# cr1m5onk1ng/text_similarity

Hardware: AMD Instinct MI355X
Metric: sentences/sec encoded + Mpairs/sec cosine top-k @ N=1M d=384 (higher is better)
Workload: dtype bf16 encoder / f16 selection / fp32 scores

## Files before the change

include/tsim.h:

```cpp
#ifndef TSIM_H
#define TSIM_H

#include <stddef.h>
#include <stdint.h>

#ifdef __cplusplus
extern "C" {
#endif

#define TSIM_OK 0
#define TSIM_EINVAL 1
#define TSIM_EHIP 2
#define TSIM_ENOMEM 3
#define TSIM_EUNSUPPORTED 4

#define TSIM_F32 0
#define TSIM_BF16 1

#define TSIM_ARCH_BERT 0
#define TSIM_ARCH_MPNET 1
#define TSIM_ARCH_ROBERTA 2

int tsim_version(void);
const char *tsim_last_error(void);
// ... 258 lines not shown
void tsim_encoder_destroy(tsim_encoder *enc);

int tsim_encoder_forward(tsim_encoder *enc, const int32_t *tok_ids, const int32_t *tok_pos,
                         const int32_t *tok_col, const int32_t *cu_seqlens, int32_t T, int32_t B,
                         int32_t max_len, float *pooled_f32, void *unit_f16, int ld_unit, float *unit_rho_max,
                         void *last_hidden_bf16, void *stream);

int tsim_encoder_set_token_types(tsim_encoder *enc, const float *type_emb_host, int32_t n_types);
int tsim_encoder_set_cls_head(tsim_encoder *enc, const float *pool_w_host, const float *pool_b_host,
                              const float *cls_w_host, const float *cls_b_host, int32_t num_labels);
int tsim_encoder_set_cls_head_act(tsim_encoder *enc, const float *pool_w_host, const float *pool_b_host,
                                  const float *cls_w_host, const float *cls_b_host, int32_t num_labels, int32_t act);
int tsim_encoder_forward_ex(tsim_encoder *enc, const int32_t *tok_ids, const int32_t *tok_type, const int32_t *tok_pos,
                            const int32_t *tok_col, const int32_t *cu_seqlens, int32_t T, int32_t B, int32_t max_len,
                            float *pooled_f32, void *unit_f16, int ld_unit, float *unit_rho_max,
                            void *last_hidden_bf16, float *logits_f32, void *stream);

#define TSIM_POOL_MEAN 0
#define TSIM_POOL_CLS 1
#define TSIM_POOL_MAX 2
#define TSIM_POOL_MEAN_SQRT_LEN 3
#define TSIM_ACT_IDENTITY 0
#define TSIM_ACT_TANH 1
#define TSIM_ACT_RELU 2
typedef struct tsim_sentence_head {
    int32_t pool_mode;
    int32_t d_out;
    const float *dense_w, *dense_b;
    int32_t dense_act;
    int32_t normalize;
} tsim_sentence_head;

int tsim_encoder_forward_head(tsim_encoder *enc, const int32_t *tok_ids, const int32_t *tok_type, const int32_t *tok_pos,
                              const int32_t *tok_col, const int32_t *cu_seqlens, int32_t T, int32_t B, int32_t max_len,
                              const tsim_sentence_head *head, float *emb_f32, void *unit_f16, int ld_unit,
                              float *unit_rho_max, void *last_hidden_bf16, void *stream);

int tsim_encoder_forward_spans(tsim_encoder *enc, const int32_t *tok_ids, const int32_t *tok_type, const int32_t *tok_pos,
                               const int32_t *tok_col, const int32_t *cu_seqlens, int32_t T, int32_t B, int32_t max_len,
                               float *pooled_f32, void *unit_f16, int ld_unit, float *unit_rho_max,
                               void *last_hidden_bf16, float *logits_f32, const int32_t *span_seq, const int32_t *span_cu,
                               const int32_t *span_tok, int32_t S, int32_t n_span_tok, float *span_out_f32,
                               void *span_unit_f16, int ld_span_unit, float *span_rho_max, void *stream);

#define TSIM_ENC_ERR_TOKEN_ID 1
#define TSIM_ENC_ERR_POSITION 2
#define TSIM_ENC_ERR_MAX_LEN 4
#define TSIM_ENC_ERR_TOKEN_TYPE 8
#define TSIM_ENC_ERR_SPAN 16
int tsim_encoder_error_flags(tsim_encoder *enc, int32_t *flags_host, void *stream);

int tsim_chain_items_host(int blocks, int rem_blocks, int ntiles, int G, int b, int32_t *items, int cap);

#define TSIM_FAMILY_H64 0
#define TSIM_FAMILY_H384_PACKED 1
#define TSIM_FAMILY_H384_ROWMAJOR 2
#define TSIM_FAMILY_PP 3
#define TSIM_FAMILY_PP_MX 4
#define TSIM_ROUTE_QKV 0
#define TSIM_ROUTE_O 1
#define TSIM_ROUTE_FFN1 2
#define TSIM_ROUTE_FFN2 3
#define TSIM_FORM_BF16_128x64 1
#define TSIM_FORM_BF16_128x128 2
#define TSIM_FORM_XRES2 3
#define TSIM_FORM_XRES2_PACKED 4
#define TSIM_FORM_PP_256_PACKED_W 5
#define TSIM_FORM_PP_256 6
#define TSIM_FORM_PP_128 7
#define TSIM_FORM_PP_MX 8
#define TSIM_FORM_BF16_RES_LN 9
#define TSIM_FORM_LN384 10
#define TSIM_FORM_PP_RES_LN_PACKED_W 11
#define TSIM_FORM_PP_RES_LN 12
#define TSIM_FORM_PP_MX_RES_LN 13
#define TSIM_SEG_LN_ROWS 1
#define TSIM_SEG_LN_ROWS_CHAINED 2
#define TSIM_SEG_LN_TAIL 3
#define TSIM_SEG_LN_SPLIT2 4
#define TSIM_SEG_LN_SPLIT4 5
#define TSIM_SEG_BF16_128x384 6
#define TSIM_SEG_BF16_64x384 7
#define TSIM_IMG_PP_QKV_O 1
#define TSIM_IMG_LN_KTILE 2
#define TSIM_IMG_LN_FRAG 4
#define TSIM_IMG_MXFP8 8
#define TSIM_BUF_YBUF 1
#define TSIM_BUF_LNIMG 2
#define TSIM_BUF_MX_ACT 4
#define TSIM_ROUTE_MAX_SEGS 4

typedef struct tsim_route_segment {
    int32_t form, row0, rows;
} tsim_route_segment;

typedef struct tsim_encoder_route {
    int32_t family;
    int32_t form[4];
    int32_t images;
    int32_t buffers;
    int32_t chain_blocks;
    int32_t qkv_chained;
    int32_t n_seg[2];
    tsim_route_segment seg[2][TSIM_ROUTE_MAX_SEGS];
} tsim_encoder_route;

// ... 15 lines not shown
```

text_similarity_amd/_lib.py:

```python
from __future__ import annotations

import ctypes as C
import os

_HERE = os.path.dirname(os.path.abspath(__file__))
LIB_PATH = os.environ.get("TSIM_LIB") or os.path.join(_HERE, "libtsim.so")

TSIM_F32, TSIM_BF16 = 0, 1
TSIM_I32, TSIM_I64 = 2, 3
LIST_ST_ROW, LIST_ST_LIMS = 1, 2
IVF_ST_LIST, IVF_ST_OFF = 1, 2
COMMUNITY_ST_ROW, COMMUNITY_ST_LIMS = 1, 2
IVF_SEG = 512
IVFPQ_SEG = 4096
GRAPH_ST_ROW, GRAPH_ST_ITERS = 1, 2
GRAPH_MAX_TABLE_BYTES = 131072
GRAPH_STATIC_LDS_BYTES = 18432
GRAPH_MAX_COARSE_LISTS = 4096
GRAPH_INSERT_ST_ROW = 1
GRAPH_LINK_POOL = 256
GRAPH_LINK_ST_CUT, GRAPH_LINK_ST_ROW, GRAPH_LINK_ST_LIMS = 1, 2, 4
ARCH_BERT, ARCH_MPNET, ARCH_ROBERTA = 0, 1, 2
W_BF16, W_MXFP8 = 0, 1
POOL_MEAN, POOL_CLS, POOL_MAX, POOL_MEAN_SQRT_LEN = 0, 1, 2, 3
# ... 151 lines not shown
                                     C.c_void_p, C.c_void_p, C.c_size_t, C.c_void_p]),
    "tsim_ivfpq_tables_workspace_bytes": (C.c_size_t, [C.c_int64, C.c_int]),
    "tsim_ivfpq_tables": (C.c_int, [C.c_int, C.c_void_p, C.c_int64, C.c_int64, C.c_void_p, C.c_int64, C.c_int64, C.c_void_p, C.c_int,
                                    C.c_void_p, C.c_int, C.c_int, C.c_void_p, C.c_void_p, C.c_void_p, C.c_void_p, C.c_size_t,
                                    C.c_void_p]),
    "tsim_ivfpq_scan_workspace_bytes": (C.c_size_t, [C.c_int64, C.c_int, C.c_int64, C.c_int]),
    "tsim_ivfpq_scan_topk": (C.c_int, [C.c_int, C.c_void_p, C.c_int, C.c_void_p, C.c_int64, C.c_void_p, C.c_int64, C.c_int64, C.c_int,
                                       C.c_void_p, C.c_int64, C.c_void_p, C.c_void_p, C.c_int, C.c_int64, C.c_int, C.c_void_p,
                                       C.c_void_p, C.c_int64, C.c_void_p, C.c_void_p, C.c_size_t, C.c_void_p]),
    "tsim_graph_search_lds_bytes": (C.c_size_t, [C.c_int, C.c_int, C.c_int, C.c_int]),
    "tsim_graph_search": (C.c_int, [C.c_int, C.c_void_p, C.c_int64, C.c_int64, C.c_void_p, C.c_int64, C.c_int64, C.c_int, C.c_void_p,
                                    C.c_int, C.c_void_p, C.c_int, C.c_void_p, C.c_int, C.c_int, C.c_int, C.c_int, C.c_void_p, C.c_void_p,
                                    C.c_int64, C.c_void_p, C.c_void_p]),
    "tsim_graph_search_seeded": (C.c_int, [C.c_int, C.c_void_p, C.c_int64, C.c_int64, C.c_void_p, C.c_int64, C.c_int64, C.c_int,
                                           C.c_void_p, C.c_int, C.c_void_p, C.c_int64, C.c_int, C.c_void_p, C.c_int64, C.c_int,
                                           C.c_void_p, C.c_int64, C.c_void_p, C.c_int, C.c_int, C.c_int, C.c_int, C.c_void_p,
                                           C.c_void_p, C.c_int64, C.c_void_p, C.c_void_p, C.c_void_p]),
    "tsim_graph_prune": (C.c_int, [C.c_void_p, C.c_int64, C.c_int, C.c_int, C.c_void_p, C.c_void_p, C.c_void_p]),
    "tsim_community_select_workspace_bytes": (C.c_size_t, [C.c_int64, C.c_int64]),
    "tsim_community_select_rounds": (C.c_int, [C.c_void_p, C.c_void_p, C.c_int64, C.c_int64, C.c_int64, C.c_int, C.c_int64, C.c_int,
                                               C.c_void_p, C.c_void_p, C.c_void_p, C.c_void_p, C.c_void_p, C.c_size_t, C.c_void_p]),
    "tsim_community_select_finish": (C.c_int, [C.c_void_p, C.c_void_p, C.c_int64, C.c_int64, C.c_int64, C.c_int, C.c_void_p,
                                               C.c_void_p, C.c_void_p, C.c_void_p, C.c_void_p, C.c_size_t, C.c_void_p]),
    "tsim_mst_prim_workspace_bytes": (C.c_size_t, [C.c_int64]),
    "tsim_mst_prim": (C.c_int, [C.c_void_p, C.c_int64, C.c_int64, C.c_int, C.c_void_p, C.c_void_p, C.c_void_p, C.c_void_p, C.c_void_p,
                                C.c_size_t, C.c_void_p]),
    "tsim_hdbscan_tree_labels": (C.c_int, [C.c_void_p, C.c_void_p, C.c_void_p, C.c_int64, C.c_int, C.c_void_p, C.c_void_p]),
    "tsim_cosine_topk": (C.c_int, [C.c_void_p, C.c_int64, C.c_void_p, C.c_int64, C.c_int, C.c_int, C.c_int,
                                   C.c_void_p, C.c_void_p, C.c_int64, C.c_void_p, C.c_size_t, C.c_void_p]),
    "tsim_time_next_topk": (None, [C.c_void_p, C.c_void_p]),
    "tsim_topk_merge": (C.c_int, [C.c_void_p, C.c_void_p, C.c_int, C.c_int64, C.c_int, C.c_int, C.c_void_p,
                                  C.c_void_p, C.c_void_p]),
    "tsim_topk_merge_strided": (C.c_int, [C.c_void_p, C.c_void_p, C.c_int, C.c_int64, C.c_int, C.c_int, C.c_int64, C.c_int64,
                                          C.c_void_p, C.c_void_p, C.c_void_p]),
    "tsim_wordpiece_create": (C.c_int, [C.c_char_p, C.c_void_p, C.c_int32, C.c_char_p, C.c_int32, C.c_void_p, C.c_int32, C.c_void_p,
                                        C.c_int32, C.c_int32, C.c_int32, C.c_char_p, C.c_void_p, C.c_int32, C.POINTER(C.c_void_p)]),
    "tsim_wordpiece_destroy": (None, [C.c_void_p]),
    "tsim_wordpiece_encode": (C.c_int, [C.c_void_p, C.c_char_p, C.c_void_p, C.c_int64, C.c_int32, C.c_int32, C.c_void_p, C.c_int64,
                                        C.c_void_p, C.c_void_p]),
    "tsim_cos_sim": (C.c_int, [C.c_void_p, C.c_int64, C.c_void_p, C.c_int64, C.c_int, C.c_void_p, C.c_void_p]),
    "tsim_mean_pool": (C.c_int, [C.c_void_p, C.c_int, C.c_void_p, C.c_int64, C.c_int, C.c_int, C.c_void_p,
                                 C.c_void_p]),
    "tsim_pool": (C.c_int, [C.c_void_p, C.c_int, C.c_void_p, C.c_int64, C.c_int, C.c_int, C.c_int, C.c_void_p, C.c_void_p]),
    "tsim_dense_rows": (C.c_int, [C.c_void_p, C.c_int64, C.c_int, C.c_void_p, C.c_void_p, C.c_int, C.c_int, C.c_int, C.c_void_p,
                                  C.c_void_p]),
    "tsim_quantize_mxfp8": (C.c_int, [C.c_void_p, C.c_int64, C.c_int, C.c_void_p, C.c_void_p, C.c_void_p]),
    "tsim_gemm_mxfp8": (C.c_int, [C.c_void_p, C.c_void_p, C.c_void_p, C.c_void_p, C.c_void_p, C.c_void_p, C.c_int, C.c_int,
                                  C.c_int, C.c_void_p]),
    "tsim_encoder_create": (C.c_int, [C.POINTER(EncoderConfigC), C.POINTER(EncoderWeightsC),
                                      C.POINTER(C.c_void_p)]),
    "tsim_encoder_destroy": (None, [C.c_void_p]),
    "tsim_encoder_error_flags": (C.c_int, [C.c_void_p, C.POINTER(C.c_int32), C.c_void_p]),
    "tsim_chain_items_host": (C.c_int, [C.c_int, C.c_int, C.c_int, C.c_int, C.c_int, C.POINTER(C.c_int32), C.c_int]),
    "tsim_encoder_route_host": (C.c_int, [C.POINTER(EncoderConfigC), C.c_int32, C.c_int32, C.POINTER(EncoderRouteC)]),
    "tsim_encoder_forward": (C.c_int, [C.c_void_p, C.c_void_p, C.c_void_p, C.c_void_p, C.c_void_p, C.c_int32,
                                       C.c_int32, C.c_int32, C.c_void_p, C.c_void_p, C.c_int, C.c_void_p, C.c_void_p,
                                       C.c_void_p]),
    "tsim_encoder_set_token_types": (C.c_int, [C.c_void_p, C.c_void_p, C.c_int32]),
    "tsim_encoder_set_cls_head": (C.c_int, [C.c_void_p, C.c_void_p, C.c_void_p, C.c_void_p, C.c_void_p, C.c_int32]),
    "tsim_encoder_set_cls_head_act": (C.c_int, [C.c_void_p, C.c_void_p, C.c_void_p, C.c_void_p, C.c_void_p, C.c_int32, C.c_int32]),
    "tsim_encoder_forward_ex": (C.c_int, [C.c_void_p, C.c_void_p, C.c_void_p, C.c_void_p, C.c_void_p, C.c_void_p, C.c_int32,
                                          C.c_int32, C.c_int32, C.c_void_p, C.c_void_p, C.c_int, C.c_void_p, C.c_void_p,
                                          C.c_void_p, C.c_void_p]),
    "tsim_encoder_forward_head": (C.c_int, [C.c_void_p, C.c_void_p, C.c_void_p, C.c_void_p, C.c_void_p, C.c_void_p, C.c_int32,
                                            C.c_int32, C.c_int32, C.POINTER(SentenceHeadC), C.c_void_p, C.c_void_p, C.c_int,
                                            C.c_void_p, C.c_void_p, C.c_void_p]),
    "tsim_encoder_forward_spans": (C.c_int, [C.c_void_p, C.c_void_p, C.c_void_p, C.c_void_p, C.c_void_p, C.c_void_p, C.c_int32,
                                             C.c_int32, C.c_int32, C.c_void_p, C.c_void_p, C.c_int, C.c_void_p, C.c_void_p,
                                             C.c_void_p, C.c_void_p, C.c_void_p, C.c_void_p, C.c_int32, C.c_int32, C.c_void_p,
                                             C.c_void_p, C.c_int, C.c_void_p, C.c_void_p]),
}

DECLARED_SYMBOLS = tuple(_SIGS)

_GRAPH_INSERT_SIGS = {
    "tsim_graph_insert_prune": (C.c_int, [C.c_void_p, C.c_int64, C.c_int, C.c_void_p, C.c_int64, C.c_int, C.c_void_p, C.c_void_p,
                                          C.c_void_p, C.c_void_p]),
    "tsim_graph_link_reverse": (C.c_int, [C.c_int, C.c_void_p, C.c_int64, C.c_int64, C.c_int, C.c_void_p, C.c_int, C.c_void_p,
                                          C.c_int64, C.c_void_p, C.c_void_p, C.c_void_p, C.c_void_p]),
}
GRAPH_INSERT_SYMBOLS = tuple(_GRAPH_INSERT_SIGS)


def lib() -> C.CDLL:
    global _lib
    if _lib is None:
        if not os.path.exists(LIB_PATH):
            raise TsimError(f"{LIB_PATH} not found: build it with `python -m text_similarity_amd.build` "
                            "(hipcc --offload-arch=gfx950); there is no CPU fallback")
        L = C.CDLL(LIB_PATH)
        for name, (res, args) in {**_SIGS, **_GRAPH_INSERT_SIGS}.items():
            try:
                fn = getattr(L, name)
            except AttributeError:
                def fn(*a, _n=name, **kw):
                    raise TsimError(f"libtsim.so does not export {_n}: rebuild with python -m text_similarity_amd.build")
                setattr(L, name, fn)
                continue
            fn.restype = res
            fn.argtypes = args
        _lib = L
    return _lib


def check(rc: int, what: str = "") -> None:
    if rc != 0:
# ... 4 lines not shown
```

text_similarity_amd/csrc/encoder.hip:

```cpp
#include <math.h>
#include <cmath>

#include <stdlib.h>
#include <string.h>

#include <vector>

#include <type_traits>
#include <utility>

#include "common.h"
#include "gemm_pp.h"

namespace tsim {

__device__ __forceinline__ int64_t packed_off(int64_t t, int f, int W) {
    return ((t >> 5) * (W >> 3) + (f >> 3)) * 256 + (t & 31) * 8 + (f & 7);
}
__device__ __forceinline__ int64_t group_off(int64_t t, int g, int W, int packed) {
    return packed ? packed_off(t, 8 * g, W) * 2 : (t * W + 8 * g) * 2;
}

template <int VPL, bool TYPED = false>
__global__ __launch_bounds__(256) void embed_ln_kernel(const int32_t *__restrict__ ids,
// ... 870 lines not shown
    constexpr int NW = 8, N = 384, LR_NST = 3;
    constexpr int LSTAGE = NW * 32 * LR_BK * 2 + LR_WBYTES;
    typedef X2Loop<EPI, true, true, true, X2Chain> Loop;
    constexpr int BMX = Loop::BMX;
    constexpr int BIAS_OFF = X2_NSTAGE * Loop::STAGE, GB_OFF = BIAS_OFF + 6144;
    static_assert(LR_NST * LSTAGE <= BIAS_OFF && Loop::NW == NW && 2 * Loop::PPW + 24 <= 63, "hand-over layout");
    extern __shared__ __attribute__((aligned(16))) char smem[];
    const int lane = threadIdx.x & 63;
    const int wave = __builtin_amdgcn_readfirstlane(threadIdx.x >> 6);
    const int m0l = blockIdx.x * BMX;

    for (int p = wave; p * 256 < N2; p += NW)
        if (p * 256 + lane * 4 < N2) glds16(bias2 + p * 256 + lane * 4, smem + BIAS_OFF + p * 1024);
    if (wave < 2 && wave * 256 + lane * 4 < N) {
        glds16(gamma + wave * 256 + lane * 4, smem + GB_OFF + wave * 1024);
        glds16(beta + wave * 256 + lane * 4, smem + GB_OFF + N * 4 + wave * 1024);
    }

    f32x16 acc[12];
    ln384_bias_start(acc, lbias, lane >> 5);
    ln384_kloop<NW, LR_NST, false>(acc, X, Wimg, smem, wave, lane, lane & 31, lane >> 5, m0l, M, K, xpacked);
    wait_vmcnt<0>();
    __builtin_amdgcn_s_barrier();

    const int ntiles = N2 / X2_BN, G = (int)gridDim.x, wg = (int)blockIdx.x;
    const X2Chain items{chain_part(G, rem_blocks, ntiles, wg), G, ntiles, wg};
    Loop x2(xout, W2, out2, smem, BIAS_OFF, M, N2, wave, items, items.part.n, wg);
    x2.prime(__builtin_amdgcn_mbcnt_hi(~0u, __builtin_amdgcn_mbcnt_lo(~0u, 0u)));

    {
        const int lane1 = __builtin_amdgcn_mbcnt_hi(~0u, __builtin_amdgcn_mbcnt_lo(~0u, 0u));
        ln384_add_residual(acc, res, (uint32_t)group_off(m0l + wave * 32 + (lane1 & 31), lane1 >> 5, N, respacked),
                           (uint32_t)group_off(0, 1, N, respacked));
        float mean, rstd;
        ln384_stats(acc, eps, mean, rstd);
        int lane3 = __builtin_amdgcn_mbcnt_hi(~0u, __builtin_amdgcn_mbcnt_lo(~0u, 0u));
        asm volatile("" : "+v"(lane3));
        const uint32_t oo = (uint32_t)group_off(m0l + wave * 32 + (lane3 & 31), lane3 >> 5, N, 1);
        constexpr uint32_t ogs = 512;
        const uint64_t xb = (uint64_t)(uintptr_t)xout;
        const float *gl = reinterpret_cast<const float *>(smem + GB_OFF);
        ln384_normalise(acc, mean, rstd, gl, gl + N, lane3 >> 5, [&](int g, const u32x4 &o) __attribute__((always_inline)) {
            x2_store16(oo + g * ogs, o, xb);
            x2.bx[g / 2] = __builtin_bit_cast(bf16x8, o);
        });
    }

    int lane2 = __builtin_amdgcn_mbcnt_hi(~0u, __builtin_amdgcn_mbcnt_lo(~0u, 0u));
    asm volatile("" : "+v"(lane2));
    x2.start(lane2);
    x2.run();
}

template <int DH, bool REL, bool PK = false>
__global__ __launch_bounds__(256) __attribute__((amdgpu_waves_per_eu(DH <= 32 ? 6 : 4))) void attention_kernel(const bf16_t *__restrict__ qkv,
                                                        const int32_t *__restrict__ cu, const int32_t *__restrict__ col,
                                                        const float *__restrict__ relb, int relw, int H,
                                                        int heads, float scale, bf16_t *__restrict__ ctx, int B, int xcd_map) {
    constexpr int KS = DH / 16;
    constexpr int OT = (DH + 31) / 32;
    constexpr int ROWB = DH * 2 < 64 ? 64 : DH * 2;
    __shared__ __attribute__((aligned(16))) char vimg[4 * 32 * ROWB];
    typedef __attribute__((ext_vector_type(4))) short s16x4;
    const int lane = threadIdx.x & 63;
    const int wave = __builtin_amdgcn_readfirstlane(threadIdx.x >> 6);
    int seq = blockIdx.x;
    if (xcd_map) {
        seq = (blockIdx.x & 7) * (gridDim.x >> 3) + (blockIdx.x >> 3);
        if (seq >= B) return;
    }
    const int head = blockIdx.y * 4 + wave, qb = blockIdx.z;
    const int t0 = cu[seq], S = cu[seq + 1] - t0;
    if (qb * 32 >= S || head >= heads) return;
    const int r = lane & 31, h = lane >> 5;
    const int64_t H3 = 3 * (int64_t)H;
    const int qi = qb * 32 + r;
    const int tq = t0 + (qi < S ? qi : S - 1);

    bf16x8 qf[KS];
    {
        const bf16_t *qp = PK ? qkv + packed_off(tq, head * DH + 8 * h, (int)H3) : qkv + tq * H3 + head * DH + 8 * h;
#pragma unroll
        for (int s = 0; s < KS; ++s) {
            qf[s] = *reinterpret_cast<const bf16x8 *>(qp + (PK ? 2 * 256 : 16) * s);
        }
    }
    const int qcol = REL ? col[tq] : 0;
    f32x16 o[OT];
#pragma unroll
    for (int ob = 0; ob < OT; ++ob)
#pragma unroll
        for (int g = 0; g < 16; ++g) o[ob][g] = 0.f;
    float m = -INFINITY, l = 0.f;

    for (int k0 = 0; k0 < S; k0 += 32) {
        const int kr = k0 + r;
        const int tk = t0 + (kr < S ? kr : S - 1);
        f32x16 sc;
#pragma unroll
        for (int g = 0; g < 16; ++g) sc[g] = 0.f;
        constexpr int CH = DH / 16;
        uint4 vr[CH];
        {
            const bf16_t *kp = PK ? qkv + packed_off(tk, H + head * DH + 8 * h, (int)H3) : qkv + tk * H3 + H + head * DH + 8 * h;
            const bf16_t *vsrc = PK ? qkv + packed_off(tk, 2 * H + head * DH + h * (DH / 2), (int)H3)
                                    : qkv + tk * H3 + 2 * H + head * DH + h * (DH / 2);
            bf16x8 kf[KS];
#pragma unroll
            for (int s = 0; s < KS; ++s) kf[s] = *reinterpret_cast<const bf16x8 *>(kp + (PK ? 2 * 256 : 16) * s);
#pragma unroll
            for (int c = 0; c < CH; ++c) vr[c] = *reinterpret_cast<const uint4 *>(vsrc + (PK ? 256 : 8) * c);
#pragma unroll
            for (int s = 0; s < KS; ++s) sc = __builtin_amdgcn_mfma_f32_32x32x16_bf16(kf[s], qf[s], sc, 0, 0, 0);
        }
        float bm = -INFINITY;
#pragma unroll
        for (int g = 0; g < 16; ++g) {
            const int key = k0 + (g & 3) + 8 * (g >> 2) + 4 * h;
            float v = sc[g] * scale;
            if (REL) {
                const int kc = col[t0 + (key < S ? key : S - 1)];
                v += relb[head * relw + (kc - qcol) + (relw >> 1)];
            }
            v = key < S ? v : -INFINITY;
            sc[g] = v;
            bm = fmaxf(bm, v);
// ... 11 lines not shown
        l = l * corr + ps;
        m = mn;
#pragma unroll
        for (int ob = 0; ob < OT; ++ob)
#pragma unroll
            for (int g = 0; g < 16; ++g) o[ob][g] *= corr;
        bf16x8 pf[2];
#pragma unroll
        for (int s = 0; s < 2; ++s)
#pragma unroll
            for (int j = 0; j < 8; ++j) pf[s][j] = (__bf16)sc[8 * s + j];
        {
            char *vrow = vimg + wave * (32 * ROWB) + r * ROWB + h * DH;
#pragma unroll
            for (int c = 0; c < CH; ++c) *reinterpret_cast<uint4 *>(vrow + 16 * c) = vr[c];
        }
        __builtin_amdgcn_wave_barrier();
#pragma unroll
        for (int ob = 0; ob < OT; ++ob) {
            const bool iv = ob * 32 + r < DH;
            const int grp16 = (lane >> 4) & 1, q4 = (lane & 15) >> 2, p4 = lane & 3;
#pragma unroll
            for (int s = 0; s < 2; ++s) {
                bf16x8 vf;
#pragma unroll
                for (int half = 0; half < 2; ++half) {
                    const int key = 16 * s + 8 * half + 4 * h + q4;
                    const char *ad = vimg + wave * (32 * ROWB) + key * ROWB + (ob * 32 + grp16 * 16 + 4 * p4) * 2;
                    const s16x4 t = __builtin_amdgcn_ds_read_tr16_b64_v4i16((__attribute__((address_space(3))) s16x4 *)ad);
#pragma unroll
                    for (int e = 0; e < 4; ++e)
                        vf[4 * half + e] = __builtin_bit_cast(__bf16, (bf16_t)(iv ? (bf16_t)t[e] : (bf16_t)0));
                }
                o[ob] = __builtin_amdgcn_mfma_f32_32x32x16_bf16(vf, pf[s], o[ob], 0, 0, 0);
            }
        }
        __builtin_amdgcn_wave_barrier();
    }
    if (qi < S) {
        const float inv = 1.0f / l;
        bf16_t *op = ctx + (int64_t)(t0 + qi) * H + head * DH + 4 * h;
#pragma unroll
        for (int ob = 0; ob < OT; ++ob)
#pragma unroll
            for (int gq = 0; gq < 4; ++gq) {
                const int i = ob * 32 + 8 * gq;
                if (i + 4 * h < DH) {
                    uint2 w;
                    w.x = pack_bf16x2(o[ob][4 * gq] * inv, o[ob][4 * gq + 1] * inv);
                    w.y = pack_bf16x2(o[ob][4 * gq + 2] * inv, o[ob][4 * gq + 3] * inv);
                    *reinterpret_cast<uint2 *>(op + i) = w;
                }
            }
    }
}

template <int NP, int MODE = TSIM_POOL_MEAN, bool NORM = false>
__global__ __launch_bounds__(256) void pool_packed_kernel(const bf16_t *__restrict__ x,
                                                          const int32_t *__restrict__ cu, int B, int H,
                                                          float *__restrict__ pooled, unit_t *__restrict__ unit,
                                                          int ld_unit, float *__restrict__ rho_max) {
    __shared__ __attribute__((aligned(16))) float rows[4][NP * 512];
    const int lane = threadIdx.x & 63, w = threadIdx.x >> 6;
    const int b = blockIdx.x * 4 + w;
    if (b >= B) return;
    const int t0 = cu[b], t1 = cu[b + 1];
    float s[NP][8];
#pragma unroll
    for (int p = 0; p < NP; ++p)
#pragma unroll
        for (int e = 0; e < 8; ++e) s[p][e] = MODE == TSIM_POOL_MAX ? -INFINITY : 0.f;
    auto add_row = [&](int p, const uint4 &v) __attribute__((always_inline)) {
        const uint32_t wv[4] = {v.x, v.y, v.z, v.w};
#pragma unroll
        for (int q = 0; q < 4; ++q) {
            s[p][2 * q] += __uint_as_float(wv[q] << 16);
            s[p][2 * q + 1] += __uint_as_float(wv[q] & 0xffff0000u);
        }
    };
    if constexpr (MODE == TSIM_POOL_CLS) {
#pragma unroll
        for (int p = 0; p < NP; ++p) {
            const int f0 = (lane + 64 * p) * 8;
            if (f0 >= H || t1 <= t0) continue;
            const uint4 v = *reinterpret_cast<const uint4 *>(x + (int64_t)t0 * H + f0);
            const uint32_t wv[4] = {v.x, v.y, v.z, v.w};
#pragma unroll
            for (int q = 0; q < 4; ++q) {
                s[p][2 * q] = __uint_as_float(wv[q] << 16);
                s[p][2 * q + 1] = __uint_as_float(wv[q] & 0xffff0000u);
            }
        }
    } else if constexpr (MODE == TSIM_POOL_MAX) {
#pragma unroll
        for (int p = 0; p < NP; ++p) {
            const int f0 = (lane + 64 * p) * 8;
            if (f0 >= H) continue;
            const bf16_t *xp = x + f0;
            for (int t = t0; t < t1; t += 8) {
                uint4 v[8];
#pragma unroll
                for (int u = 0; u < 8; ++u) v[u] = *reinterpret_cast<const uint4 *>(xp + (int64_t)(t + u < t1 ? t + u : t1 - 1) * H);
#pragma unroll
                for (int u = 0; u < 8; ++u) {
                    const uint32_t wv[4] = {v[u].x, v[u].y, v[u].z, v[u].w};
#pragma unroll
// ... 781 lines not shown
    hipLaunchKernelGGL(kern, dim3((unsigned)blocks), dim3(512), lds, st, g.X, g.Wf, g.bias, g.res, g.gamma, g.beta, g.eps, g.out, g.K,
                       (int)g.lay.x, (int)g.lay.res, W2, bias2, out2, M, N2, rem_blocks);
    TSIM_HIP_CHECK(hipGetLastError());
    return TSIM_OK;
}

static int ln384_gemm(const LnGemm &g, int T, bool chained, float *lnimg, hipStream_t st) {
    tsim_route_segment seg[TSIM_ROUTE_MAX_SEGS];
    const int n = ln384_segments(T, g.K, chained, seg);
    for (int i = 0; i < n; ++i) {
        const int r0 = seg[i].row0, rows = seg[i].rows;
        LnGemm s = g;
        s.X += (int64_t)r0 * g.K, s.res += (int64_t)r0 * 384, s.out += (int64_t)r0 * 384;
        int rc = TSIM_OK;
        switch (seg[i].form) {
            case TSIM_SEG_LN_ROWS_CHAINED: break;
            case TSIM_SEG_LN_ROWS: rc = ln_rows_gemm<8, 3>(s, rows, st); break;
            case TSIM_SEG_BF16_128x384:
                rc = launch_gemm<128, 384, 64, 2, 4, EPI_RES_LN>(s.X, s.W, s.bias, s.res, s.gamma, s.beta, s.eps, s.out, rows, 384, s.K, st, s.Wk, s.lay);
                break;
            case TSIM_SEG_BF16_64x384:
                rc = launch_gemm<64, 384, 64, 2, 4, EPI_RES_LN>(s.X, s.W, s.bias, s.res, s.gamma, s.beta, s.eps, s.out, rows, 384, s.K, st, s.Wk, s.lay);
                break;
            default: rc = ln_tail_gemm(s, rows, seg[i].form, lnimg, st);
        }
        if (rc) return rc;
    }
    return TSIM_OK;
}

template <int V>
using int_c = std::integral_constant<int, V>;

static int embed_rows(tsim_encoder *e, const int32_t *tok_ids, const int32_t *tok_type, const int32_t *tok_pos, const int32_t *tok_col,
                      int T, int max_len, hipStream_t st) {
    const tsim_encoder_config &c = e->cfg;
    const int32_t *colp = tok_col ? tok_col : tok_pos;
    const int col_limit = tok_col || c.arch == TSIM_ARCH_BERT ? max_len : c.max_pos;
    auto launch = [&](auto kern) {
        hipLaunchKernelGGL(kern, dim3((unsigned)((T + 3) / 4)), dim3(256), 0, st, tok_ids, tok_pos, e->word, e->pos, e->type0, e->emb_g, e->emb_b,
                           c.ln_eps, T, c.hidden, e->x0, c.vocab, c.max_pos, colp, col_limit, e->err_flags, tok_type, tok_type ? e->n_types : 0);
    };
    auto go = [&](auto v) { tok_type ? launch(embed_ln_kernel<decltype(v)::value, true>) : launch(embed_ln_kernel<decltype(v)::value, false>); };
    c.hidden == 64 ? go(int_c<1>{}) : c.hidden == 384 ? go(int_c<6>{}) : c.hidden == 768 ? go(int_c<12>{}) : go(int_c<16>{});
    TSIM_HIP_CHECK(hipGetLastError());
    return TSIM_OK;
}

struct Forward {
    tsim_encoder *e;
    const int32_t *cu_seqlens, *col;
    int T, B, H, F, chain;
    float eps;
    dim3 agrid;
    hipStream_t st;
    using Layer = tsim_encoder::Layer;

    int attention() const {
        const int heads = e->cfg.heads, dh = H / heads;
        auto launch = [&](auto kern) {
            hipLaunchKernelGGL(kern, agrid, dim3(256), 0, st, e->qkv, cu_seqlens, col, e->relb, e->relw, H, heads, 1.0f / sqrtf((float)dh), e->ctx, B, 1);
        };
        auto go = [&](auto d) {
            constexpr int D = decltype(d)::value;
            if (e->cfg.arch == TSIM_ARCH_MPNET) launch(attention_kernel<D, true, false>);
            else if (e->plan.family == TSIM_FAMILY_H384_PACKED) launch(attention_kernel<D, false, true>);
            else launch(attention_kernel<D, false, false>);
        };
        dh == 16 ? go(int_c<16>{}) : dh == 32 ? go(int_c<32>{}) : go(int_c<64>{});
        TSIM_HIP_CHECK(hipGetLastError());
        return TSIM_OK;
    }

    int ffn1_rowmajor(const Layer &L) const {
        switch (const int form = e->plan.form[TSIM_ROUTE_FFN1]) {
            case TSIM_FORM_XRES2: return gemm_xres2<EPI_GELU, false, false>(e->x1, L.w1, L.b1, e->h1, T, F, st);
            case TSIM_FORM_PP_256: case TSIM_FORM_PP_128: return gemm_pp(PP_EPI_GELU, e->x1, L.w1, 0, L.b1, e->h1, T, F, H, st);
            case TSIM_FORM_BF16_128x128:
                return launch_gemm<128, 128, 64, 2, 2, EPI_GELU>(e->x1, L.w1, L.b1, nullptr, nullptr, nullptr, 0.f, e->h1, T, F, H, st, nullptr, ALL_ROW_MAJOR);
            case TSIM_FORM_BF16_128x64:
                return launch_gemm<128, 64, 64, 2, 2, EPI_GELU>(e->x1, L.w1, L.b1, nullptr, nullptr, nullptr, 0.f, e->h1, T, F, H, st, nullptr, ALL_ROW_MAJOR);
            default: return fail(TSIM_EINVAL, "encoder: FFN1 form %d is not a row-major one", form);
        }
    }

    int layer_mx(int l) const {
        const Layer &L = e->layers[l];
        int rc;
        if (l == 0 && (rc = quant_mx(e->x0, T, H, e->aq, e->as, st))) return rc;
        if ((rc = gemm_pp_mx(PP_EPI_BIAS, e->aq, e->as, L.qqkv, 1, L.sqkv, L.bqkv, e->qkv, nullptr, T, 3 * H, H, st))) return rc;
        if ((rc = attention()) || (rc = quant_mx(e->ctx, T, H, e->aq, e->as, st))) return rc;
        if ((rc = gemm_pp_mx(PP_EPI_F32, e->aq, e->as, L.qo, 1, L.so, L.bo, e->ybuf, nullptr, T, H, H, st))) return rc;
        if ((rc = res_ln_rows(e->ybuf, e->x0, L.g1, L.be1, eps, e->x1, e->aq, e->as, T, H, st))) return rc;
        if ((rc = gemm_pp_mx(PP_EPI_GELU_MX, e->aq, e->as, L.q1, 1, L.s1, L.b1, e->hq, e->hs, T, F, H, st))) return rc;
        if ((rc = gemm_pp_mx(PP_EPI_F32, e->hq, e->hs, L.q2, 1, L.s2, L.b2, e->ybuf, nullptr, T, H, F, st))) return rc;
        return res_ln_rows(e->ybuf, e->x1, L.g2, L.be2, eps, e->x0, e->aq, e->as, T, H, st);
    }

    int layer_pp(int l) const {
        const Layer &L = e->layers[l];
        const bool pq = e->plan.form[TSIM_ROUTE_QKV] == TSIM_FORM_PP_256_PACKED_W, po = e->plan.form[TSIM_ROUTE_O] == TSIM_FORM_PP_RES_LN_PACKED_W;
        int rc;
        if ((rc = gemm_pp(PP_EPI_BIAS, e->x0, pq ? L.pqkv : L.wqkv, pq, L.bqkv, e->qkv, T, 3 * H, H, st)) || (rc = attention())) return rc;
        if ((rc = gemm_pp(PP_EPI_F32, e->ctx, po ? L.po : L.wo, po, L.bo, e->ybuf, T, H, H, st))) return rc;
        if ((rc = res_ln_rows(e->ybuf, e->x0, L.g1, L.be1, eps, e->x1, nullptr, nullptr, T, H, st)) || (rc = ffn1_rowmajor(L))) return rc;
        if ((rc = gemm_pp(PP_EPI_F32, e->h1, L.w2, 0, L.b2, e->ybuf, T, H, F, st))) return rc;
        return res_ln_rows(e->ybuf, e->x1, L.g2, L.be2, eps, e->x0, nullptr, nullptr, T, H, st);
    }

    int layer_384(int l) const {
        const Layer &L = e->layers[l];
        const bool pk = e->plan.family == TSIM_FAMILY_H384_PACKED, last = l + 1 == e->cfg.num_layers, chain_qkv = chain > 0 && !last;
        const Layout packed = pk ? BLOCK_PACKED : ROW_MAJOR, x0_in = pk && l > 0 ? BLOCK_PACKED : ROW_MAJOR, x0_out = pk && !last ? BLOCK_PACKED : ROW_MAJOR;
        int rc;
// ... 9 lines not shown
        if (rc) return rc;
        const LnGemm f2 = {e->h1, L.w2, L.l2, L.l232, L.b2, e->x1, L.g2, L.be2, eps, e->x0, F, {packed, packed, x0_out}};
        if ((rc = ln384_gemm(f2, T, chain_qkv, e->lnimg, st)) || !chain_qkv) return rc;
        return ln_rows_xres2<EPI_BIAS>(f2, chain, e->layers[l + 1].wqkv, e->layers[l + 1].bqkv, e->qkv, T, 3 * H, st);
    }

    int layer_h64(int l) const {
        const Layer &L = e->layers[l];
        int rc;
        if ((rc = launch_gemm<128, 64, 64, 2, 2, EPI_BIAS>(e->x0, L.wqkv, L.bqkv, nullptr, nullptr, nullptr, 0.f, e->qkv, T, 3 * H, H, st, nullptr, ALL_ROW_MAJOR))) return rc;
        if ((rc = attention()) || (rc = launch_gemm<128, 64, 64, 4, 2, EPI_RES_LN>(e->ctx, L.wo, L.bo, e->x0, L.g1, L.be1, eps, e->x1, T, H, H, st, nullptr, ALL_ROW_MAJOR))) return rc;
        if ((rc = ffn1_rowmajor(L))) return rc;
        return launch_gemm<128, 64, 64, 4, 2, EPI_RES_LN>(e->h1, L.w2, L.b2, e->x1, L.g2, L.be2, eps, e->x0, T, H, F, st, nullptr, ALL_ROW_MAJOR);
    }
};

static int pool_rows(const tsim_encoder *e, const int32_t *cu_seqlens, int B, int mode, bool norm, float *px, unit_t *pu, int ld_unit,
                     float *unit_rho_max, hipStream_t st) {
    const int H = e->cfg.hidden;
    auto launch = [&](auto kern) {
        hipLaunchKernelGGL(kern, dim3((unsigned)((B + 3) / 4)), dim3(256), 0, st, e->x0, cu_seqlens, B, H, px, pu, ld_unit, pu ? unit_rho_max : nullptr);
    };
    auto by_width = [&](auto m, auto n) {
        H <= 512 ? launch(pool_packed_kernel<1, decltype(m)::value, decltype(n)::value>) : launch(pool_packed_kernel<2, decltype(m)::value, decltype(n)::value>);
    };
    auto by_mode = [&](auto n) {
        mode == TSIM_POOL_MEAN ? by_width(int_c<TSIM_POOL_MEAN>{}, n) : mode == TSIM_POOL_CLS ? by_width(int_c<TSIM_POOL_CLS>{}, n)
        : mode == TSIM_POOL_MAX ? by_width(int_c<TSIM_POOL_MAX>{}, n) : by_width(int_c<TSIM_POOL_MEAN_SQRT_LEN>{}, n);
    };
    norm ? by_mode(std::true_type{}) : by_mode(std::false_type{});
    TSIM_HIP_CHECK(hipGetLastError());
    return TSIM_OK;
}

static int cls_head(const tsim_encoder *e, const int32_t *cu_seqlens, int B, float *logits_f32, hipStream_t st) {
    const int H = e->cfg.hidden;
    auto launch = [&](auto kern) {
        hipLaunchKernelGGL(kern, dim3((unsigned)((B + CLS_ROWS - 1) / CLS_ROWS)), dim3((unsigned)H), 0, st, e->x0, cu_seqlens, B, H, e->head_wpT,
                           e->head_bp, e->head_wc, e->head_bc, e->n_labels, logits_f32);
    };
    if (e->head_act == TSIM_ACT_RELU) H <= CLS_MAX_H ? launch(cls_head_wide_kernel<CLS_MAX_H, TSIM_ACT_RELU>) : launch(cls_head_wide_kernel<CLS_WIDE_H, TSIM_ACT_RELU>);
    else H <= CLS_MAX_H ? launch(cls_head_kernel) : launch(cls_head_wide_kernel<CLS_WIDE_H, TSIM_ACT_TANH>);
    TSIM_HIP_CHECK(hipGetLastError());
    return TSIM_OK;
}

}

extern "C" int tsim_chain_items_host(int blocks, int rem_blocks, int ntiles, int G, int b, int32_t *items, int cap) {
    if (blocks != G || rem_blocks < 0 || ntiles <= 0 || G <= 0 || b < 0 || b >= G || (cap > 0 && !items)) return -1;
    const ChainPart p = chain_part(G, rem_blocks, ntiles, b);
    for (int i = 0; i < p.n && i < cap; ++i) items[i] = chain_item(p, G, ntiles, b, i);
    return p.n;
}

extern "C" int tsim_encoder_route_host(const tsim_encoder_config *cfg, int32_t T, int32_t layer, tsim_encoder_route *out) {
    TSIM_REQUIRE(cfg && out, "encoder_route_host: null pointer");
    TSIM_REQUIRE(T >= 0 && layer >= 0 && layer < cfg->num_layers, "encoder_route_host: T=%d layer=%d of %d", T, layer, cfg->num_layers);
    if (int rc = encoder_plan(*cfg, out)) return rc;
    out->chain_blocks = chain_blocks(*out, cfg->ffn, T);
    out->qkv_chained = out->chain_blocks > 0 && layer > 0;
    if (out->form[TSIM_ROUTE_O] == TSIM_FORM_LN384) {
        out->n_seg[0] = ln384_segments(T, cfg->hidden, out->chain_blocks > 0, out->seg[0]);
        out->n_seg[1] = ln384_segments(T, cfg->ffn, out->chain_blocks > 0 && layer + 1 < cfg->num_layers, out->seg[1]);
    }
    return TSIM_OK;
}

extern "C" int tsim_encoder_create(const tsim_encoder_config *cfg, const tsim_encoder_weights_host *w,
                                   tsim_encoder **out) {
    TSIM_REQUIRE(cfg && w && out, "encoder_create: null pointer");
    EncoderPlan plan;
    if (int rc = encoder_plan(*cfg, &plan)) return rc;
    const int H = cfg->hidden, F = cfg->ffn, L = cfg->num_layers;
    TSIM_REQUIRE(w->word_emb && w->pos_emb && w->emb_ln_g && w->emb_ln_b && w->layers, "encoder_create: missing weights");
    TSIM_REQUIRE(cfg->arch != TSIM_ARCH_MPNET || w->rel_bias, "encoder_create: MPNet needs rel_bias");
    const bool mx = plan.images & TSIM_IMG_MXFP8;
    tsim_encoder *e = new tsim_encoder();
    e->cfg = *cfg;
    e->plan = plan;
    e->Tp = (cfg->max_tokens + 127) / 128 * 128 + 128;
    int rc = TSIM_OK;
    auto bail = [&](int code) {
        tsim_encoder_destroy(e);
        return code;
    };
    if ((rc = upload_f32(e, w->word_emb, (size_t)cfg->vocab * H, &e->word))) return bail(rc);
    if ((rc = upload_f32(e, w->pos_emb, (size_t)cfg->max_pos * H, &e->pos))) return bail(rc);
    if (w->type_emb && (rc = upload_f32(e, w->type_emb, H, &e->type0))) return bail(rc);
    if ((rc = upload_f32(e, w->emb_ln_g, H, &e->emb_g))) return bail(rc);
    if ((rc = upload_f32(e, w->emb_ln_b, H, &e->emb_b))) return bail(rc);
    if (cfg->arch == TSIM_ARCH_MPNET) {
        const int maxp = cfg->max_pos;
        e->relw = 2 * maxp - 1;
        std::vector<float> tab((size_t)cfg->heads * e->relw);
        for (int d = -(maxp - 1); d <= maxp - 1; ++d) {
            const int bk = mpnet_bucket(d, cfg->rel_buckets);
            for (int hh = 0; hh < cfg->heads; ++hh) tab[(size_t)hh * e->relw + d + maxp - 1] = w->rel_bias[bk * cfg->heads + hh];
        }
        if ((rc = upload_f32(e, tab.data(), tab.size(), &e->relb))) return bail(rc);
    }
    e->layers.resize(L);
    for (int l = 0; l < L; ++l) {
        const tsim_layer_weights_host &lw = w->layers[l];
        tsim_encoder::Layer &d = e->layers[l];
        if ((rc = upload_bf16(e, {lw.wq, lw.wk, lw.wv}, (size_t)H * H, &d.wqkv))) return bail(rc);
// ... 138 lines not shown
    TSIM_REQUIRE(e->cfg.arch != TSIM_ARCH_MPNET, "encoder_set_cls_head: BERT only");
    TSIM_REQUIRE(act == TSIM_ACT_TANH || act == TSIM_ACT_RELU, "encoder_set_cls_head: activation %d (TSIM_ACT_TANH, TSIM_ACT_RELU)", act);
    TSIM_REQUIRE(num_labels >= 1 && num_labels <= CLS_MAX_LABELS, "encoder_set_cls_head: num_labels=%d outside [1, %d]", num_labels,
                 CLS_MAX_LABELS);
    const int H = e->cfg.hidden;
    TSIM_REQUIRE(H % 64 == 0 && H <= CLS_WIDE_H, "encoder_set_cls_head: hidden=%d unsupported", H);
    std::vector<float> wT((size_t)H * H);
    for (int o = 0; o < H; ++o)
        for (int k = 0; k < H; ++k) wT[(size_t)k * H + o] = pool_w_host[(size_t)o * H + k];
    int rc;
    if ((rc = upload_f32(e, wT.data(), wT.size(), &e->head_wpT))) return rc;
    if ((rc = upload_f32(e, pool_b_host, H, &e->head_bp))) return rc;
    if ((rc = upload_f32(e, cls_w_host, (size_t)num_labels * H, &e->head_wc))) return rc;
    if ((rc = upload_f32(e, cls_b_host, num_labels, &e->head_bc))) return rc;
    e->n_labels = num_labels;
    e->head_act = act;
    return TSIM_OK;
}

extern "C" int tsim_encoder_forward(tsim_encoder *e, const int32_t *tok_ids, const int32_t *tok_pos,
                                    const int32_t *tok_col, const int32_t *cu_seqlens, int32_t T, int32_t B,
                                    int32_t max_len, float *pooled_f32, void *unit_bf16, int ld_unit, float *unit_rho_max,
                                    void *last_hidden_bf16, void *stream) {
    return tsim_encoder_forward_ex(e, tok_ids, nullptr, tok_pos, tok_col, cu_seqlens, T, B, max_len, pooled_f32, unit_bf16, ld_unit,
                                   unit_rho_max, last_hidden_bf16, nullptr, stream);
}

extern "C" int tsim_encoder_forward_ex(tsim_encoder *e, const int32_t *tok_ids, const int32_t *tok_type, const int32_t *tok_pos,
                                       const int32_t *tok_col, const int32_t *cu_seqlens, int32_t T, int32_t B,
                                       int32_t max_len, float *pooled_f32, void *unit_bf16, int ld_unit, float *unit_rho_max,
                                       void *last_hidden_bf16, float *logits_f32, void *stream) {
    TSIM_REQUIRE(e && cu_seqlens && (T == 0 || (tok_ids && tok_pos)), "encoder_forward: null pointer");
    TSIM_REQUIRE(!tok_type || e->n_types > 0, "encoder_forward: tok_type given but no token-type table was set "
                 "(tsim_encoder_set_token_types)");
    TSIM_REQUIRE(!logits_f32 || e->n_labels > 0, "encoder_forward: logits requested but no classification head was set "
                 "(tsim_encoder_set_cls_head)");
    TSIM_REQUIRE(T >= 0 && B >= 0 && T <= e->cfg.max_tokens && B <= e->cfg.max_seqs,
                 "encoder_forward: T=%d B=%d exceed capacity (%d tokens, %d sequences)", T, B, e->cfg.max_tokens, e->cfg.max_seqs);
    const int pos_span = max_len + (e->cfg.arch != TSIM_ARCH_BERT ? e->cfg.pad_id + 1 : 0);
    TSIM_REQUIRE(max_len >= 0 && pos_span <= e->cfg.max_pos,
                 "encoder_forward: sequences of %d tokens need position rows up to %d, the table has %d", max_len, pos_span - 1,
                 e->cfg.max_pos);
    TSIM_REQUIRE(!unit_bf16 || ld_unit >= e->cfg.hidden, "encoder_forward: ld_unit < hidden");
    TSIM_REQUIRE(!unit_bf16 || e->cfg.hidden <= 768, "encoder_forward: unit rows need a width <= 768 (got %d)", e->cfg.hidden);
    if (B == 0) return TSIM_OK;
    hipStream_t st = reinterpret_cast<hipStream_t>(stream);
    const tsim_encoder_config &c = e->cfg;
    const int H = c.hidden;
    int rc;
    if (T > 0) {
        if ((rc = embed_rows(e, tok_ids, tok_type, tok_pos, tok_col, T, max_len, st))) return rc;
        const int qblocks = (max_len + 31) / 32 > 0 ? (max_len + 31) / 32 : 1;
        const Forward f = {e, cu_seqlens, c.arch == TSIM_ARCH_MPNET ? (tok_col ? tok_col : tok_pos) : nullptr, T, B, H, c.ffn, chain_blocks(e->plan, c.ffn, T),
                           c.ln_eps, dim3((unsigned)(((B + 7) / 8) * 8), (unsigned)((c.heads + 3) / 4), (unsigned)qblocks), st};
        for (int l = 0; l < c.num_layers; ++l) {
            switch (e->plan.family) {
                case TSIM_FAMILY_PP_MX: rc = f.layer_mx(l); break;
                case TSIM_FAMILY_PP: rc = f.layer_pp(l); break;
                case TSIM_FAMILY_H64: rc = f.layer_h64(l); break;
                default: rc = f.layer_384(l);
            }
            if (rc) return rc;
        }
        if (last_hidden_bf16)
            TSIM_HIP_CHECK(hipMemcpyAsync(last_hidden_bf16, e->x0, (size_t)T * H * 2, hipMemcpyDeviceToDevice, st));
    }
    if (pooled_f32 || unit_bf16) {
        if (H % 8 != 0 || H > 1024 || (unit_bf16 && ld_unit % 8 != 0))
            return fail(TSIM_EUNSUPPORTED, "encoder: pooling needs a hidden size that is a multiple of 8, at most 1024 (got %d)", H);
        if (((uintptr_t)pooled_f32 | (uintptr_t)unit_bf16) & 15)
            return fail(TSIM_EINVAL, "encoder: pooled / unit outputs must be 16-byte aligned");
        if ((rc = pool_rows(e, cu_seqlens, B, TSIM_POOL_MEAN, false, pooled_f32, (unit_t *)unit_bf16, ld_unit, unit_rho_max, st))) return rc;
    }
    if (logits_f32) return cls_head(e, cu_seqlens, B, logits_f32, st);
    return TSIM_OK;
}

extern "C" int tsim_encoder_forward_head(tsim_encoder *e, const int32_t *tok_ids, const int32_t *tok_type, const int32_t *tok_pos,
                                         const int32_t *tok_col, const int32_t *cu_seqlens, int32_t T, int32_t B, int32_t max_len,
                                         const tsim_sentence_head *head, float *emb_f32, void *unit_f16, int ld_unit,
                                         float *unit_rho_max, void *last_hidden_bf16, void *stream) {
    if (!head)
        return tsim_encoder_forward_ex(e, tok_ids, tok_type, tok_pos, tok_col, cu_seqlens, T, B, max_len, emb_f32, unit_f16, ld_unit,
                                       unit_rho_max, last_hidden_bf16, nullptr, stream);
    TSIM_REQUIRE(e, "encoder_forward_head: null encoder");
    const int H = e->cfg.hidden, mode = head->pool_mode, d_out = head->d_out;
    TSIM_REQUIRE(mode >= TSIM_POOL_MEAN && mode <= TSIM_POOL_MEAN_SQRT_LEN, "encoder_forward_head: unknown pool_mode %d", mode);
    TSIM_REQUIRE(head->normalize == 0 || head->normalize == 1, "encoder_forward_head: normalize=%d is not 0 / 1", head->normalize);
    TSIM_REQUIRE(d_out >= 0, "encoder_forward_head: d_out=%d < 0", d_out);
    if (d_out) {
        TSIM_REQUIRE(head->dense_w, "encoder_forward_head: d_out=%d without dense_w", d_out);
        if (int rc = dense_check(H, d_out, head->dense_act, head->dense_w)) return rc;
    } else {
        TSIM_REQUIRE(!head->dense_w && !head->dense_b, "encoder_forward_head: dense weights given with d_out = 0");
    }
    const int width = d_out ? d_out : H;
    TSIM_REQUIRE(!unit_f16 || width <= 768, "encoder_forward_head: unit rows need a final width <= 768 (got %d)", width);
    TSIM_REQUIRE(!unit_f16 || (ld_unit >= width && ld_unit % 8 == 0), "encoder_forward_head: ld_unit=%d (final width %d)", ld_unit,
                 width);
    TSIM_REQUIRE(H % 8 == 0 && H <= 1024, "encoder_forward_head: pooling needs hidden %% 8 == 0 and <= 1024 (got %d)", H);
    TSIM_REQUIRE((((uintptr_t)emb_f32 | (uintptr_t)unit_f16) & 15) == 0, "encoder_forward_head: outputs must be 16-byte aligned");
    if (int rc = tsim_encoder_forward_ex(e, tok_ids, tok_type, tok_pos, tok_col, cu_seqlens, T, B, max_len, nullptr, nullptr, 0,
                                         nullptr, last_hidden_bf16, nullptr, stream))
        return rc;
    if (B == 0 || (!emb_f32 && !unit_f16)) return TSIM_OK;
    hipStream_t st = reinterpret_cast<hipStream_t>(stream);
    float *px = d_out ? (e->head_x ? e->head_x : reinterpret_cast<float *>(e->qkv)) : emb_f32;
// ... 21 lines not shown
```

Measured before the change: 883,200.

## Pack upper query blocks of several sequences into one attention workgroup

The attention launch changes from a 3D grid (sequence x head-group x query-block) to a flat 1D grid. The first query block of every sequence still gets its own workgroup. Query blocks beyond the first are grouped so that one workgroup walks up to G sequences, using a ballot over sequence lengths to pick only those long enough to need that block. The goal is to remove the many empty workgroups that launch and exit at once when sequences are shorter than max_len. The cost is serialised work inside a workgroup and added index arithmetic. A host mapping function is exported for testing.

```diff
diff --git a/include/tsim.h b/include/tsim.h
--- a/include/tsim.h
+++ b/include/tsim.h
@@ -334,6 +334,8 @@
 
 int tsim_chain_items_host(int blocks, int rem_blocks, int ntiles, int G, int b, int32_t *items, int cap);
 
+int64_t tsim_attention_map_host(int B, int heads, int max_len, int64_t block0, int n, int32_t *out);
+
 #define TSIM_FAMILY_H64 0
 #define TSIM_FAMILY_H384_PACKED 1
 #define TSIM_FAMILY_H384_ROWMAJOR 2
diff --git a/text_similarity_amd/_lib.py b/text_similarity_amd/_lib.py
--- a/text_similarity_amd/_lib.py
+++ b/text_similarity_amd/_lib.py
@@ -227,6 +227,7 @@
     "tsim_encoder_destroy": (None, [C.c_void_p]),
     "tsim_encoder_error_flags": (C.c_int, [C.c_void_p, C.POINTER(C.c_int32), C.c_void_p]),
     "tsim_chain_items_host": (C.c_int, [C.c_int, C.c_int, C.c_int, C.c_int, C.c_int, C.POINTER(C.c_int32), C.c_int]),
+    "tsim_attention_map_host": (C.c_int64, [C.c_int, C.c_int, C.c_int, C.c_int64, C.c_int, C.POINTER(C.c_int32)]),
     "tsim_encoder_route_host": (C.c_int, [C.POINTER(EncoderConfigC), C.c_int32, C.c_int32, C.POINTER(EncoderRouteC)]),
     "tsim_encoder_forward": (C.c_int, [C.c_void_p, C.c_void_p, C.c_void_p, C.c_void_p, C.c_void_p, C.c_int32,
                                        C.c_int32, C.c_int32, C.c_void_p, C.c_void_p, C.c_int, C.c_void_p, C.c_void_p,
diff --git a/text_similarity_amd/csrc/encoder.hip b/text_similarity_amd/csrc/encoder.hip
--- a/text_similarity_amd/csrc/encoder.hip
+++ b/text_similarity_amd/csrc/encoder.hip
@@ -946,26 +946,46 @@
     x2.run();
 }
 
-template <int DH, bool REL, bool PK = false>
-__global__ __launch_bounds__(256) __attribute__((amdgpu_waves_per_eu(DH <= 32 ? 6 : 4))) void attention_kernel(const bf16_t *__restrict__ qkv,
-                                                        const int32_t *__restrict__ cu, const int32_t *__restrict__ col,
-                                                        const float *__restrict__ relb, int relw, int H,
-                                                        int heads, float scale, bf16_t *__restrict__ ctx, int B, int xcd_map) {
+#ifndef TSIM_ATT_GROUP
+#define TSIM_ATT_GROUP 8
+#define TSIM_ATT_GROUP_MIN_WGS 8192
+#endif
+constexpr int ATT_GROUP = TSIM_ATT_GROUP, ATT_GROUP_MIN_WGS = TSIM_ATT_GROUP_MIN_WGS;
+struct AttShape { int nb8, hgs, planes, G, ngx; };
+struct AttSlot { int upper, seq0, n, hg, qb; };
+__host__ __device__ inline AttShape att_shape(int B, int heads, int planes) {
+    const int nb8 = (B + 7) / 8, hgs = (heads + 3) / 4;
+    const int G = (long long)nb8 * 8 * hgs * planes >= ATT_GROUP_MIN_WGS ? ATT_GROUP : 1;
+    return {nb8, hgs, planes, G, (nb8 + G - 1) / G};
+}
+__host__ __device__ inline long long att_upper_blocks(const AttShape &a) { return 8LL * a.ngx * a.hgs * (a.planes - 1); }
+__host__ __device__ inline long long att_grid(const AttShape &a) { return att_upper_blocks(a) + 8LL * a.nb8 * a.hgs; }
+__host__ __device__ inline AttSlot att_slot(const AttShape &a, int B, int b) {
+    const int U = (int)att_upper_blocks(a), x = b & 7;
+    if (b < U) {
+        const int i = b >> 3, qb = 1 + i % (a.planes - 1), hg = i / (a.planes - 1) % a.hgs, j = i / (a.planes - 1) / a.hgs;
+        const int s0 = x * a.nb8 + j * a.G, s1 = x * a.nb8 + (j * a.G + a.G < a.nb8 ? j * a.G + a.G : a.nb8);
+        const int n = (s1 < B ? s1 : B) - s0;
+        return {1, s0, n > 0 ? n : 0, hg, qb};
+    }
+    const int f = b - U, bx = f % (8 * a.nb8), seq = x * a.nb8 + (bx >> 3);
+    return {0, seq, seq < B ? 1 : 0, f / (8 * a.nb8), 0};
+}
+
+template <int DH>
+struct AttVImage {
+    static constexpr int ROWB = DH * 2 < 64 ? 64 : DH * 2;
+    static constexpr int BYTES = 4 * 32 * ROWB;
+};
+
+template <int DH, bool REL, bool PK>
+__device__ __forceinline__ void attention_block(const bf16_t *__restrict__ qkv, const int32_t *__restrict__ col,
+                                                const float *__restrict__ relb, int relw, int H, float scale, bf16_t *__restrict__ ctx,
+                                                char *vimg, int lane, int wave, int head, int qb, int t0, int S) {
     constexpr int KS = DH / 16;
     constexpr int OT = (DH + 31) / 32;
-    constexpr int ROWB = DH * 2 < 64 ? 64 : DH * 2;
-    __shared__ __attribute__((aligned(16))) char vimg[4 * 32 * ROWB];
+    constexpr int ROWB = AttVImage<DH>::ROWB;
     typedef __attribute__((ext_vector_type(4))) short s16x4;
-    const int lane = threadIdx.x & 63;
-    const int wave = __builtin_amdgcn_readfirstlane(threadIdx.x >> 6);
-    int seq = blockIdx.x;
-    if (xcd_map) {
-        seq = (blockIdx.x & 7) * (gridDim.x >> 3) + (blockIdx.x >> 3);
-        if (seq >= B) return;
-    }
-    const int head = blockIdx.y * 4 + wave, qb = blockIdx.z;
-    const int t0 = cu[seq], S = cu[seq + 1] - t0;
-    if (qb * 32 >= S || head >= heads) return;
     const int r = lane & 31, h = lane >> 5;
     const int64_t H3 = 3 * (int64_t)H;
     const int qi = qb * 32 + r;
@@ -1083,6 +1103,31 @@
                     *reinterpret_cast<uint2 *>(op + i) = w;
                 }
             }
+    }
+}
+
+template <int DH, bool REL, bool PK = false>
+__global__ __launch_bounds__(256) __attribute__((amdgpu_waves_per_eu(DH <= 32 ? 6 : 4))) void attention_kernel(const bf16_t *__restrict__ qkv,
+                                                        const int32_t *__restrict__ cu, const int32_t *__restrict__ col,
+                                                        const float *__restrict__ relb, int relw, int H,
+                                                        int heads, float scale, bf16_t *__restrict__ ctx, int B, int planes) {
+    __shared__ __attribute__((aligned(16))) char vimg[AttVImage<DH>::BYTES];
+    const int lane = threadIdx.x & 63;
+    const int wave = __builtin_amdgcn_readfirstlane(threadIdx.x >> 6);
+    const AttSlot slot = att_slot(att_shape(B, heads, planes), B, (int)blockIdx.x);
+    const int head = slot.hg * 4 + wave, qb = slot.qb;
+    if (slot.n == 0 || head >= heads) return;
+    unsigned long long todo = 1;
+    if (slot.upper) {
+        const int s = slot.seq0 + (lane < slot.n ? lane : 0);
+        todo = __ballot(lane < slot.n && cu[s + 1] - cu[s] > qb * 32);
+    }
+    for (; todo; todo &= todo - 1) {
+        const int seq = slot.seq0 + __builtin_ctzll(todo);
+        const int t0 = cu[seq], S = cu[seq + 1] - t0;
+        int lane1;
+        asm volatile("v_mbcnt_lo_u32_b32 %0, -1, 0\n\tv_mbcnt_hi_u32_b32 %0, -1, %0" : "=v"(lane1));
+        if (qb * 32 < S) attention_block<DH, REL, PK>(qkv, col, relb, relw, H, scale, ctx, vimg, lane1, wave, head, qb, t0, S);
     }
 }
 
@@ -1970,14 +2015,16 @@
     const int32_t *cu_seqlens, *col;
     int T, B, H, F, chain;
     float eps;
-    dim3 agrid;
+    int planes;
     hipStream_t st;
     using Layer = tsim_encoder::Layer;
 
     int attention() const {
         const int heads = e->cfg.heads, dh = H / heads;
+        const long long grid = att_grid(att_shape(B, heads, planes));
+        if (grid > INT32_MAX) return fail(TSIM_EINVAL, "encoder: attention over %d sequences x %d query blocks needs %lld workgroups", B, planes, grid);
         auto launch = [&](auto kern) {
-            hipLaunchKernelGGL(kern, agrid, dim3(256), 0, st, e->qkv, cu_seqlens, col, e->relb, e->relw, H, heads, 1.0f / sqrtf((float)dh), e->ctx, B, 1);
+            hipLaunchKernelGGL(kern, dim3((unsigned)grid), dim3(256), 0, st, e->qkv, cu_seqlens, col, e->relb, e->relw, H, heads, 1.0f / sqrtf((float)dh), e->ctx, B, planes);
         };
         auto go = [&](auto d) {
             constexpr int D = decltype(d)::value;
@@ -2093,6 +2140,19 @@
     const ChainPart p = chain_part(G, rem_blocks, ntiles, b);
     for (int i = 0; i < p.n && i < cap; ++i) items[i] = chain_item(p, G, ntiles, b, i);
     return p.n;
+}
+
+extern "C" int64_t tsim_attention_map_host(int B, int heads, int max_len, int64_t block0, int n, int32_t *out) {
+    if (B <= 0 || heads <= 0 || max_len < 0 || n < 0 || (n > 0 && !out)) return -1;
+    const AttShape a = att_shape(B, heads, (max_len + 31) / 32 > 0 ? (max_len + 31) / 32 : 1);
+    const long long grid = att_grid(a);
+    if (grid > INT32_MAX || block0 < 0 || block0 + n > grid) return -1;
+    for (int i = 0; i < n; ++i) {
+        const AttSlot s = att_slot(a, B, (int)block0 + i);
+        const int32_t v[6] = {s.upper, s.seq0, s.n, s.hg, s.qb, a.G};
+        for (int k = 0; k < 6; ++k) out[6 * i + k] = v[k];
+    }
+    return grid;
 }
 
 extern "C" int tsim_encoder_route_host(const tsim_encoder_config *cfg, int32_t T, int32_t layer, tsim_encoder_route *out) {
@@ -2337,7 +2397,7 @@
         if ((rc = embed_rows(e, tok_ids, tok_type, tok_pos, tok_col, T, max_len, st))) return rc;
         const int qblocks = (max_len + 31) / 32 > 0 ? (max_len + 31) / 32 : 1;
         const Forward f = {e, cu_seqlens, c.arch == TSIM_ARCH_MPNET ? (tok_col ? tok_col : tok_pos) : nullptr, T, B, H, c.ffn, chain_blocks(e->plan, c.ffn, T),
-                           c.ln_eps, dim3((unsigned)(((B + 7) / 8) * 8), (unsigned)((c.heads + 3) / 4), (unsigned)qblocks), st};
+                           c.ln_eps, qblocks, st};
         for (int l = 0; l < c.num_layers; ++l) {
             switch (e->plan.family) {
                 case TSIM_FAMILY_PP_MX: rc = f.layer_mx(l); break;
```

Result: no change. 886,300, median of 6 (+0.4%).
